# timohouben/GNN-XAI-TimeSeries-QualityControl

Hardware: AMD Instinct MI355X
Metric: ROC-AUC (5-fold CV) + train windows/sec, CML GCN at 1/2/4/8 MI355X (higher is better)
Workload: dtype bf16; 1 GPU; model=CML GCN (GeneralConv16+mean pool+LSTM TimeLayer f16 n_stacks2+dense64), global_batch=128, seq_len=181, parallelism=dp1, adjacency=radius(max_sample_distance=20), graph_steps=8, trainable_params=188193, hip_graph=True

## Files before the change

csrc/kernels/chain_head.h:

```cpp
#pragma once
#include "common.h"

namespace gq {

constexpr int CH_HU = 64;
constexpr int CH_AP = CH_HU + 4;
constexpr int CH_NW = 8;
constexpr int CH_WP = CH_HU + 4;

struct ChainHead {
  const float *W1, *b1, *W2, *b2, *W3, *b3;
  const float *y, *mask;
  float* logits;
  float* part;
  float* loss;
  double* sums;
  float* hist;
  int bins;
  int* ticket;
  int* done;
  int* ctl;
  int M;
  float alpha1, alpha2, w0, w1;
  const float* dloss;
  float* gpart;
  float *dW1, *db1, *dW2, *db2, *dW3, *db3;
};

template <int F>
struct ChainHeadRec {
  static constexpr int N = F * CH_HU + CH_HU + CH_HU * CH_HU + CH_HU + CH_HU + 1;
  static constexpr int PITCH = (N + 3) / 4 * 4;
};

typedef float ch_f4 __attribute__((ext_vector_type(4)));

__device__ __forceinline__ void ch_st(float* p, float v) {
  __hip_atomic_store(reinterpret_cast<unsigned*>(p), __float_as_uint(v), __ATOMIC_RELAXED, __HIP_MEMORY_SCOPE_AGENT);
}
__device__ __forceinline__ float ch_ld(const float* p) {
  return __uint_as_float(__hip_atomic_load(reinterpret_cast<const unsigned*>(p), __ATOMIC_RELAXED,
                                           __HIP_MEMORY_SCOPE_AGENT));
}

__device__ __forceinline__ float ch_leaky(float z, float a) { return z > 0.f ? z : a * z; }
__device__ __forceinline__ float ch_dleaky(float z, float a) { return z > 0.f ? 1.f : a; }

__device__ __forceinline__ int ch_tid() { return threadIdx.x & (64 * CH_NW - 1); }

__device__ __forceinline__ float ch_mask_sum(const float* __restrict__ mask, int M, float* red) {
  float s = 0.f;
  for (int i = ch_tid(); i < M; i += 64 * CH_NW) s += ch_ld(mask + i);
  s = wave_sum(s);
  if ((threadIdx.x & 63) == 0) red[ch_tid() >> 6] = s;
  __syncthreads();
  float t = 0.f;
#pragma unroll
  for (int k = 0; k < CH_NW; ++k) t += red[k];
  return t;
}

template <int NS>
__device__ __forceinline__ ch_f4 ch_mm_wk(const float* __restrict__ Wt, int ldw, int ot, int k0, const float* act,
                                          int lda) {
  const int l = threadIdx.x & 63, m = l & 15, kk = l >> 4;
  float a[NS];
#pragma unroll
  for (int s = 0; s < NS; ++s) a[s] = Wt[(size_t)(k0 + 4 * s + kk) * ldw + 16 * ot + m];
  ch_f4 acc = {0.f, 0.f, 0.f, 0.f};
#pragma unroll
  for (int s = 0; s < NS; ++s)
    acc = __builtin_amdgcn_mfma_f32_16x16x4f32(a[s], act[m * lda + k0 + 4 * s + kk], acc, 0, 0, 0);
  return acc;
}

template <int NS>
__device__ __forceinline__ ch_f4 ch_mm_wt(const float* __restrict__ W, int ldw, int ot, int k0, const float* act,
                                          int lda) {
  const int l = threadIdx.x & 63, m = l & 15, kk = l >> 4;
  float a[NS];
#pragma unroll
  for (int s = 0; s < NS; ++s) a[s] = W[(size_t)(16 * ot + m) * ldw + k0 + 4 * s + kk];
  ch_f4 acc = {0.f, 0.f, 0.f, 0.f};
#pragma unroll
  for (int s = 0; s < NS; ++s)
    acc = __builtin_amdgcn_mfma_f32_16x16x4f32(a[s], act[m * lda + k0 + 4 * s + kk], acc, 0, 0, 0);
  return acc;
}

__device__ __forceinline__ void ch_put(float* part, int lp, int ot, const ch_f4& d) {
  const int l = threadIdx.x & 63, n = l & 15, q = l >> 4;
#pragma unroll
// ... 29 lines not shown
  const int tid = ch_tid(), w = tid >> 6, j = tid & 63;
  const int ot = w & 3, kh = w >> 2;
  const float b1j = hd.b1[j], b2j = hd.b2[j];
  ch_put(part + kh * PT, CH_AP, ot, ch_mm_wk<F / 8>(sW1, CH_WP, ot, kh * (F / 2), hl, HLP));
  __syncthreads();
#pragma unroll
  for (int q = 0; q < 2; ++q) {
    const int r = w + 8 * q;
    const float z1 = b1j + part[r * CH_AP + j] + part[PT + r * CH_AP + j];
    if (sz1 != nullptr) sz1[r * CH_AP + j] = z1;
    sa1[r * CH_AP + j] = ch_leaky(z1, hd.alpha1);
  }
  __syncthreads();
  ch_put(part + kh * PT, CH_AP, ot, ch_mm_wk<8>(sW2, CH_WP, ot, kh * 32, sa1, CH_AP));
  __syncthreads();
#pragma unroll
  for (int q = 0; q < 2; ++q) {
    const int r = w + 8 * q;
    z2[q] = b2j + part[r * CH_AP + j] + part[PT + r * CH_AP + j];
  }
}

template <int F>
struct ChainHeadFwdLds {
  static constexpr int BYTES = (2 * 16 * CH_AP + 16 * CH_AP + 16 * 8 + (F + CH_HU) * CH_WP) * 4;
};

template <int F>
__device__ __forceinline__ float* ch_head_fwd_weights(char* scratch) {
  return reinterpret_cast<float*>(scratch) + 3 * 16 * CH_AP + 16 * 8;
}
template <int F>
__device__ __forceinline__ void chain_head_fwd_handoff(const ChainHead hd, int tile, int ntiles, char* scratch);
template <int F>
__device__ __forceinline__ void chain_head_fwd(const ChainHead hd, int tile, int ntiles, const float* hl, char* scratch,
                                               bool staged = false, bool handoff = true) {
  float* part = reinterpret_cast<float*>(scratch);
  float* sa1 = part + 2 * 16 * CH_AP;
  float* rowv = sa1 + 16 * CH_AP;
  float* sW1 = rowv + 16 * 8;
  float* sW2 = sW1 + F * CH_WP;
  if (!staged) ch_stage_weights<F>(hd, sW1, sW2);
  const int tid = threadIdx.x, w = tid >> 6, j = tid & 63;
  const float w3j = hd.W3[j], b3 = hd.b3[0];
  float yy[2], mm[2];
#pragma unroll
  for (int q = 0; q < 2; ++q) {
    const int rc = min(tile * 16 + w + 8 * q, hd.M - 1);
    yy[q] = ch_ld(hd.y + rc);
    mm[q] = ch_ld(hd.mask + rc);
  }
  float z2[2];
  ch_head_z2<F>(hd, sW1, sW2, hl, part, nullptr, sa1, z2);
#pragma unroll
  for (int q = 0; q < 2; ++q) {
    const int r = w + 8 * q, row = tile * 16 + r;
    const float z = wave_sum(ch_leaky(z2[q], hd.alpha2) * w3j) + b3;
    if (j == 0) {
      const bool valid = row < hd.M;
      const float m = valid ? mm[q] : 0.f, y = yy[q];
      if (valid && hd.logits != nullptr) hd.logits[row] = z;
      const float l = fmaxf(z, 0.f) - z * y + log1pf(__expf(-fabsf(z)));
      const float wc = y > 0.5f ? hd.w1 : hd.w0;
      const float p = sigmoidf_fast(z);
      const bool pos = y > 0.5f, pp = p > 0.5f;
      rowv[r * 8 + 0] = m * wc * l;
      rowv[r * 8 + 1] = m;
      rowv[r * 8 + 2] = (pp && pos) ? m : 0.f;
      rowv[r * 8 + 3] = (!pp && !pos) ? m : 0.f;
      rowv[r * 8 + 4] = (pp && !pos) ? m : 0.f;
      rowv[r * 8 + 5] = (!pp && pos) ? m : 0.f;
      if (hd.hist != nullptr && m != 0.f) {
        int b = (int)rintf(fminf(fmaxf(p, 0.f), 1.f) * (float)(hd.bins - 1));
        b = b < 0 ? 0 : (b >= hd.bins ? hd.bins - 1 : b);
        atomicAdd(&hd.hist[(pos ? hd.bins : 0) + b], m);
      }
    }
  }
  __syncthreads();
  if (handoff) chain_head_fwd_handoff<F>(hd, tile, ntiles, scratch);
}

template <int F>
__device__ __forceinline__ void chain_head_fwd_handoff(const ChainHead hd, int tile, int ntiles, char* scratch) {
  const float* rowv = reinterpret_cast<const float*>(scratch) + 3 * 16 * CH_AP;
  const int tid = threadIdx.x;
  if (tid < 6) {
    float s = 0.f;
#pragma unroll
    for (int k = 0; k < 16; ++k) s += rowv[k * 8 + tid];
    ch_st(hd.part + tile * 8 + tid, s);
  }
  asm volatile("s_waitcnt vmcnt(0)" ::: "memory");
  __syncthreads();
  if (tid == 0) {
    const int t = __hip_atomic_fetch_add(hd.ticket, 1, __ATOMIC_RELAXED, __HIP_MEMORY_SCOPE_AGENT);
    if (t == ntiles - 1) {
      double s[6] = {0, 0, 0, 0, 0, 0};
      for (int k = 0; k < ntiles; ++k)
        for (int q = 0; q < 6; ++q) s[q] += (double)ch_ld(hd.part + k * 8 + q);
      hd.loss[0] = (float)(s[0] / fmax(s[1], 1.0));
      if (hd.sums != nullptr)
        for (int q = 0; q < 6; ++q) hd.sums[q] += s[q];
      __hip_atomic_store(hd.ticket, 0, __ATOMIC_RELAXED, __HIP_MEMORY_SCOPE_AGENT);
    }
  }
}

template <int F>
struct ChainHeadBwdLds {
  static constexpr int BYTES = (16 * (F + 4) + 2 * 16 * CH_AP + 5 * 16 * CH_AP + 32 + (F + CH_HU) * CH_WP) * 4;
};

template <int F>
__device__ __forceinline__ void chain_head_bwd(const ChainHead hd, const float* __restrict__ hT, int tile, int ntiles,
                                               float* dh, char* scratch, int hld = -1, bool unit_gl = false,
                                               bool count = true, int nlive = 0, const float* pW1 = nullptr,
                                               const float* pW2 = nullptr) {
  constexpr int HLP = F + 4, PT = 16 * CH_AP;
  using Rec = ChainHeadRec<F>;
  float* sh = reinterpret_cast<float*>(scratch);
  float* part = sh + 16 * HLP;
  float* sz1 = part + 2 * PT;
  float* sa1 = sz1 + PT;
  float* sz2 = sa1 + PT;
  float* sad = sz2 + PT;
  float* sdz1 = sad + PT;
  float* misc = sdz1 + PT;
  float* sW1 = pW1 != nullptr ? const_cast<float*>(pW1) : misc + 32;
  float* sW2 = pW2 != nullptr ? const_cast<float*>(pW2) : sW1 + F * CH_WP;
  if (pW1 == nullptr) ch_stage_weights<F>(hd, sW1, sW2);
  const int tid = ch_tid(), w = tid >> 6, j = tid & 63;
  const int l = tid & 63, lm = l & 15, lq = l >> 4;
  const int row0 = tile * 16;
  const float* hsrc = hld < 0 ? hT + (size_t)row0 * F : hT;
  const int hp = hld < 0 ? F : hld;
  for (int e = tid; e < 16 * F / 4; e += 64 * CH_NW) {
    const int rr = 4 * e / F, k = 4 * e % F;
    const float4 v = *reinterpret_cast<const float4*>(hsrc + (size_t)rr * hp + k);
    *reinterpret_cast<float4*>(sh + rr * HLP + k) = v;
  }
  const float w3j = hd.W3[j], b3 = hd.b3[0], gl = unit_gl ? 1.f : hd.dloss[0];
  float yy[2], mm[2];
#pragma unroll
  for (int q = 0; q < 2; ++q) {
    const int rc = min(row0 + w + 8 * q, hd.M - 1);
    yy[q] = ch_ld(hd.y + rc);
    mm[q] = ch_ld(hd.mask + rc);
  }
  const float n = ch_mask_sum(hd.mask, hd.M, misc + 16);
  float z2[2];
  ch_head_z2<F>(hd, sW1, sW2, sh, part, sz1, sa1, z2);
#pragma unroll
  for (int q = 0; q < 2; ++q) {
    const int r = w + 8 * q;
    const float a2 = ch_leaky(z2[q], hd.alpha2);
    const float z = wave_sum(a2 * w3j) + b3;
    const float wc = yy[q] > 0.5f ? hd.w1 : hd.w0;
    const float d = (row0 + r < hd.M) ? gl / fmaxf(n, 1.f) * mm[q] * wc * (sigmoidf_fast(z) - yy[q]) : 0.f;
    sz2[r * CH_AP + j] = d * w3j * ch_dleaky(z2[q], hd.alpha2);
    sad[r * CH_AP + j] = a2 * d;
    if (j == 0) misc[r] = d;
  }
  __syncthreads();
  {
    const int ot = w & 3, kh = w >> 2;
    ch_put(part + kh * PT, CH_AP, ot, ch_mm_wt<8>(sW2, CH_WP, ot, kh * 32, sz2, CH_AP));
  }
  __syncthreads();
#pragma unroll
  for (int q = 0; q < 2; ++q) {
    const int r = w + 8 * q;
    const float da = part[r * CH_AP + j] + part[PT + r * CH_AP + j];
    sdz1[r * CH_AP + j] = da * ch_dleaky(sz1[r * CH_AP + j], hd.alpha1);
  }
  __syncthreads();
#pragma unroll
  for (int q = 0; q < F / 16 / CH_NW; ++q) {
    const int ot = w + CH_NW * q;
    ch_put(dh, HLP, ot, ch_mm_wt<16>(sW1, CH_WP, ot, 0, sdz1, CH_AP));
  }
  auto wgrad = [&](const float* a1, int lda1, int it, const float* a2, int jt) {
    ch_f4 acc = {0.f, 0.f, 0.f, 0.f};
#pragma unroll
    for (int s = 0; s < 4; ++s)
      acc = __builtin_amdgcn_mfma_f32_16x16x4f32(a1[(4 * s + lq) * lda1 + 16 * it + lm],
                                                 a2[(4 * s + lq) * CH_AP + 16 * jt + lm], acc, 0, 0, 0);
    return acc;
  };
  float* rec = hd.gpart + (size_t)tile * Rec::PITCH;
  float* rec2 = rec + F * CH_HU + CH_HU;
  const int wa = threadIdx.x >> 6, nwa = nlive > 0 ? nlive : (int)(blockDim.x >> 6);
  for (int t = wa; t < F / 16 * 4; t += nwa) {
    const int it = t >> 2, jt = t & 3;
    const ch_f4 acc = wgrad(sh, HLP, it, sdz1, jt);
#pragma unroll
    for (int k = 0; k < 4; ++k) ch_st(rec + (16 * it + 4 * lq + k) * CH_HU + 16 * jt + lm, acc[k]);
  }
  for (int t = wa; t < 16; t += nwa) {
    const int it = t >> 2, jt = t & 3;
    const ch_f4 acc = wgrad(sa1, CH_AP, it, sz2, jt);
#pragma unroll
    for (int k = 0; k < 4; ++k) ch_st(rec2 + (16 * it + 4 * lq + k) * CH_HU + 16 * jt + lm, acc[k]);
  }
  if (threadIdx.x < CH_HU) {
    float s1 = 0.f, s2 = 0.f, s3 = 0.f;
#pragma unroll
    for (int rr = 0; rr < 16; ++rr) {
      s1 += sdz1[rr * CH_AP + j];
      s2 += sz2[rr * CH_AP + j];
      s3 += sad[rr * CH_AP + j];
    }
    ch_st(rec + F * CH_HU + j, s1);
    ch_st(rec2 + CH_HU * CH_HU + j, s2);
    ch_st(rec2 + CH_HU * CH_HU + CH_HU + j, s3);
  } else if (threadIdx.x == CH_HU) {
    float s = 0.f;
#pragma unroll
    for (int rr = 0; rr < 16; ++rr) s += misc[rr];
    ch_st(rec2 + CH_HU * CH_HU + 2 * CH_HU, s);
  }
  if (!count) {
    __syncthreads();
    return;
  }
  asm volatile("s_waitcnt vmcnt(0)" ::: "memory");
  __syncthreads();
  if (threadIdx.x == 0) __hip_atomic_fetch_add(hd.ticket, 1, __ATOMIC_RELAXED, __HIP_MEMORY_SCOPE_AGENT);
}

template <int F>
__device__ __forceinline__ void chain_head_bwd_reduce(const ChainHead hd, int tile, int ntiles, bool pre = false,
                                                      float scale = 1.f) {
  using Rec = ChainHeadRec<F>;
  __shared__ int bad;
  if (threadIdx.x == 0 && pre) bad = 0;
  if (threadIdx.x == 0 && !pre) {
    int nap = 1, it = 0;
    bad = 0;
    while (__hip_atomic_load(hd.ticket, __ATOMIC_RELAXED, __HIP_MEMORY_SCOPE_AGENT) < ntiles) {
      for (int k = 0; k < nap; ++k) __builtin_amdgcn_s_sleep(8);
      nap = min(nap * 2, 8);
      if (++it > (1 << 22)) {
        __hip_atomic_store(hd.ctl + 2, 1, __ATOMIC_RELAXED, __HIP_MEMORY_SCOPE_AGENT);
        bad = 1;
        break;
      }
    }
  }
  __syncthreads();
  if (!bad) {
    const int chunk = (Rec::N + ntiles - 1) / ntiles;
    const int e1 = min(Rec::N, (tile + 1) * chunk);
    constexpr int RB = 4;
    for (int e0 = tile * chunk + (int)threadIdx.x; e0 < e1; e0 += RB * blockDim.x) {
      float acc[RB];
#pragma unroll
      for (int q = 0; q < RB; ++q) acc[q] = 0.f;
      for (int k = 0; k < ntiles; ++k) {
        float v[RB];
#pragma unroll
        for (int q = 0; q < RB; ++q) v[q] = ch_ld(hd.gpart + (size_t)k * Rec::PITCH + min(e0 + q * (int)blockDim.x, e1 - 1));
#pragma unroll
        for (int q = 0; q < RB; ++q) acc[q] += v[q];
      }
#pragma unroll
      for (int q = 0; q < RB; ++q) {
      const int e = e0 + q * (int)blockDim.x;
      if (e >= e1) break;
      const float s = acc[q] * scale;
      if (!isfinite(s)) __hip_atomic_store(hd.ctl + 7, 1, __ATOMIC_RELAXED, __HIP_MEMORY_SCOPE_AGENT);
      int o = e;
      if (o < F * CH_HU) { hd.dW1[o] += s; continue; }
      o -= F * CH_HU;
      if (o < CH_HU) { hd.db1[o] += s; continue; }
      o -= CH_HU;
      if (o < CH_HU * CH_HU) { hd.dW2[o] += s; continue; }
      o -= CH_HU * CH_HU;
      if (o < CH_HU) { hd.db2[o] += s; continue; }
      o -= CH_HU;
      if (o < CH_HU) { hd.dW3[o] += s; continue; }
      hd.db3[0] += s;
      }
    }
  }
  __syncthreads();
  if (threadIdx.x == 0) {
    const int d = __hip_atomic_fetch_add(hd.done, 1, __ATOMIC_ACQ_REL, __HIP_MEMORY_SCOPE_AGENT);
    if (d == ntiles - 1) {
      __hip_atomic_store(hd.ticket, 0, __ATOMIC_RELAXED, __HIP_MEMORY_SCOPE_AGENT);
      __hip_atomic_store(hd.done, 0, __ATOMIC_RELAXED, __HIP_MEMORY_SCOPE_AGENT);
    }
  }
}

}
```

csrc/kernels/lstm_chain.hip:

```cpp
#include "chain_head.h"
#include "common.h"
#include "gcn_fused.h"
#include "lstm_grads_body.h"
#include "lstm_tm_common.h"

#include <cstdlib>
#include <type_traits>

namespace gq {

typedef unsigned long long u64x2_t __attribute__((ext_vector_type(2)));
typedef unsigned u32x4_t __attribute__((ext_vector_type(4)));
typedef __bf16 bf16x2_t __attribute__((ext_vector_type(2)));

static constexpr int CHAIN_MAX = 8;
static constexpr int CHAIN_SPIN = 1 << 20;
#ifndef CHAIN_D
#define CHAIN_D 4
#endif
#ifndef CHAIN_D3
#define CHAIN_D3 2
#endif
#ifndef CHAIN_LEAD1
#define CHAIN_LEAD1 1
// ... 519 lines not shown
          stage_x((t + 1) & 1, 0, t + 1);
          if (iot == 0) chain_mark_wave(pr, t, 5);
          next_ld = t + 1 + D;
          if (iot == 0) chain_mark_wave(pr, t, 6);
        }
        kt = kt == 0 ? D - 1 : kt - 1;
        lds_barrier();
      }
    }
  } else {
    for (int t0 = 0; t0 < T; t0 += D) {
#pragma unroll
      for (int r = 0; r < D; ++r) {
        const int t = t0 + r;
        if (t >= T) break;
        compute_step(t, yes{}, (r + 1 == D) ? 0 : r + 1);
        if (own_pool && pooler && t >= 1) pool_step(t - 1);
        lds_barrier();
        chain_mark(pr, t, 3);
      }
    }
  }
  if constexpr (!IOW) {
    if (own_pool && pooler) pool_step(T - 1);
  }
}

struct ChainT4Lds {
  static constexpr int HS = 2 * 16 * (128 + 8) * 2;
  static constexpr int XS = 2 * 16 * (64 + 8) * 2;
  static constexpr int HL = 16 * (128 + 4) * 4;
  static constexpr int DHT = 16 * (128 + 4) * 4;
  static constexpr int HF = ChainHeadFwdLds<128>::BYTES;
  static constexpr int HB = DHT + ChainHeadBwdLds<128>::BYTES - (128 + CH_HU) * CH_WP * 4;
  static constexpr int BYTES = HS + XS + HL + HF + HB;
};

template <bool TRAIN>
__device__ __forceinline__ void chain_t4_stage(const ChainT4 Q, int tile, int ntiles, int Mp, unsigned tagb, int* ctl,
                                               char* smem) {
  constexpr int H = 128, G4 = 4 * H, NW = 16, CPL = 2, KX = 2, KSH = H / 32, HPB = H + 8, XP = 64 + 8;
  static_assert(ChainT4Lds::HS % 16 == 0 && ChainT4Lds::XS % 16 == 0 && ChainT4Lds::HL % 16 == 0, "t4 LDS layout");
  auto hs = reinterpret_cast<__bf16 (*)[16][HPB]>(smem);
  auto xs = reinterpret_cast<__bf16 (*)[16][XP]>(smem + ChainT4Lds::HS);
  float* hl = reinterpret_cast<float*>(smem + ChainT4Lds::HS + ChainT4Lds::XS);
  const int T = Q.T, Din = Q.Din, Dw = Q.Dw;
  const int tid = threadIdx.x, lane = tid & 63;
  const int w = __builtin_amdgcn_readfirstlane(tid >> 6);
  const int col = lane & 15, quad = lane >> 4;
  const int row0 = tile * 16;

  for (int i = tid; i < 2 * 16 * HPB; i += 1024) (&hs[0][0][0])[i] = (__bf16)0.0f;
  for (int i = tid; i < 2 * 16 * XP; i += 1024) (&xs[0][0][0])[i] = (__bf16)0.0f;
  const int n_el = 16 * Din;
  const bool own = tid < n_el;
  const int el = min(tid, n_el - 1), er = el / Din, ek = el % Din;
  const size_t xstep = (size_t)Mp * Din, xoff = (size_t)(row0 + er) * Din + ek;
  unsigned long long xq[3];
  auto load_x = [&](int tx) {
#pragma unroll
    for (int r = 0; r < 3; ++r) xq[r] = ld_granule(Q.xin + xoff + (size_t)(3 * tx + r) * xstep);
  };
  load_x(0);

  bf16x8_t ufr[CPL][KSH], wfr[CPL][KX];
  f32x4_t bias4[CPL];
  int unit[CPL];
// ... 114 lines not shown
}

__device__ __forceinline__ void chain_finish(int* ctl, int nblk) {
  if (threadIdx.x == 0) {
    const int old = __hip_atomic_fetch_add(ctl + 1, 1, __ATOMIC_RELAXED, __HIP_MEMORY_SCOPE_AGENT);
    if (old == nblk - 1) {
      __hip_atomic_store(ctl + 1, 0, __ATOMIC_RELAXED, __HIP_MEMORY_SCOPE_AGENT);
      __hip_atomic_store(ctl + 10, 0, __ATOMIC_RELAXED, __HIP_MEMORY_SCOPE_AGENT);
      __hip_atomic_fetch_add(ctl, 1, __ATOMIC_RELAXED, __HIP_MEMORY_SCOPE_AGENT);
    }
  }
}

static constexpr int CHAIN_LDS = ChainT4Lds::BYTES > CHAIN_LDS_STAGE ? ChainT4Lds::BYTES : CHAIN_LDS_STAGE;

template <bool TRAIN>
__global__ __launch_bounds__(1024) void lstm_chain_fwd_kernel(ChainArgs A) {
  const int nblk = gridDim.x;
  __shared__ __attribute__((aligned(16))) char smem[CHAIN_LDS];
  if ((int)blockIdx.x >= A.ns * A.nt8) {
    int r = (int)blockIdx.x - A.ns * A.nt8;
    if (A.t4.on) {
      if (r < A.nt8) {
        if (r < A.ntiles) {
          if (threadIdx.x == 0) A.trace[2 * blockIdx.x] = (long long)__builtin_amdgcn_s_memrealtime();
          const unsigned tagb = chain_tag_base((unsigned)__hip_atomic_load(A.ctl, __ATOMIC_RELAXED, __HIP_MEMORY_SCOPE_AGENT));
          constexpr int HOFF = ChainT4Lds::HS + ChainT4Lds::XS + ChainT4Lds::HL;
          float* hW1 = ch_head_fwd_weights<128>(smem + HOFF);
          ch_stage_weights<128>(A.t4.hd, hW1, hW1 + 128 * CH_WP);
          if (A.gp.on) {
            if (threadIdx.x == 0) chain_wait_count(A.ctl + 10, A.gp.Mp, A.ctl);
            __syncthreads();
          }
          chain_t4_stage<TRAIN>(A.t4, r, A.ntiles, A.Mp, tagb, A.ctl, smem);
          long long* mk = blockIdx.x < 64 ? A.trace + 512 + blockIdx.x : nullptr;
          if (mk != nullptr && threadIdx.x == 0) mk[0] = (long long)__builtin_amdgcn_s_memrealtime();
          if (threadIdx.x >= 64 * CH_NW) return;
          const bool pre = TRAIN && A.t4.hb != nullptr;
          chain_head_fwd<128>(A.t4.hd, r, A.ntiles, reinterpret_cast<const float*>(smem + ChainT4Lds::HS + ChainT4Lds::XS),
                              smem + HOFF, true, !pre);
          if (mk != nullptr && threadIdx.x == 0) mk[64] = (long long)__builtin_amdgcn_s_memrealtime();
          if constexpr (TRAIN) {
            if (A.t4.hb != nullptr) {
              __syncthreads();
              constexpr int OFF = HOFF + ChainT4Lds::HF;
              float* dhs = reinterpret_cast<float*>(smem + OFF);
              ChainHead hb = A.t4.hd;
              hb.gpart = A.t4.hb + (size_t)A.ntiles * 16 * 128;
              chain_head_bwd<128>(hb, reinterpret_cast<const float*>(smem + ChainT4Lds::HS + ChainT4Lds::XS), r, A.ntiles,
                                  dhs, smem + OFF + ChainT4Lds::DHT, 132, true, false, CH_NW, hW1, hW1 + 128 * CH_WP);
              for (int e = ch_tid(); e < 16 * 128; e += 64 * CH_NW)
                A.t4.hb[((size_t)r * 16 + e / 128) * 128 + e % 128] = dhs[(e / 128) * 132 + e % 128];
              chain_head_fwd_handoff<128>(A.t4.hd, r, A.ntiles, smem + HOFF);
            }
          }
          __syncthreads();
          if (threadIdx.x == 0) A.trace[2 * blockIdx.x + 1] = (long long)__builtin_amdgcn_s_memrealtime();
        }
        chain_finish(A.ctl, nblk);
        return;
      }
      r -= A.nt8;
    }
    if (r < A.npk) {
      const int f = r * 1024 + (int)threadIdx.x;
      if (A.pk != nullptr && f < T4PK_ALL) t4_pack_one(f, A.pkU, A.pkW, A.pkDw, A.pk);
    } else if (A.cf.on && r - A.npk < A.cf.Mp) {
      gcn_coef_fwd_body<2, 16>(A.cf, r - A.npk, smem);
    } else if (A.gp.on && r - A.npk - (A.cf.on ? A.cf.Mp : 0) < A.gp.Mp) {
      if (threadIdx.x == 0 && blockIdx.x < 256) A.trace[2 * blockIdx.x] = (long long)__builtin_amdgcn_s_memrealtime();
      const unsigned E = (unsigned)__hip_atomic_load(A.ctl, __ATOMIC_RELAXED, __HIP_MEMORY_SCOPE_AGENT);
      const int row = r - A.npk - (A.cf.on ? A.cf.Mp : 0);
      gcn_prod_body<2, 16>(A.gp, row, chain_tag_base(E), A.ctl + 10, smem, row < 32 ? A.trace + 640 + 4 * row : nullptr);
      if (threadIdx.x == 0 && blockIdx.x < 256) A.trace[2 * blockIdx.x + 1] = (long long)__builtin_amdgcn_s_memrealtime();
    }
    chain_finish(A.ctl, nblk);
    return;
  }
  const int s = blockIdx.x / A.nt8, tile = blockIdx.x % A.nt8;
  if (s >= A.ns || tile >= A.ntiles) {
    chain_finish(A.ctl, nblk);
    return;
  }
// ... 701 lines not shown
          const bf16x8_t bz = *reinterpret_cast<const bf16x8_t*>(&zs[p][col][32 * (kx * KPX + q) + 8 * quad]);
          b = __builtin_amdgcn_mfma_f32_16x16x32_bf16(ufk[q], bz, b, 0, 0, 0);
        }
#pragma unroll
        for (int r = 0; r < 4; ++r) {
          dpart[kg][col][16 * ut + 4 * quad + r] = a[r];
          xpart[p][kx][col][16 * xt + 4 * quad + r] = b[r];
        }
      }
      chain_mark(pr, s, 4);
      if constexpr (!PUBW) {
        const uint2 zv = *reinterpret_cast<const uint2*>(&zs[p][gz_seq][gz_c]);
        const int tz = t >= 0 ? t : T;
        *reinterpret_cast<uint2*>(zbase + (size_t)tz * zstep) = zv;
      }
      if constexpr (!PUBW) {
        const int ts = (s >= 1 && s <= T) ? t + 1 : T;
        store_dx(p ^ 1, ts, tagb | (unsigned)ts);
      }
      {
        lds_barrier();
        float sdh = 0.f;
#pragma unroll
        for (int g = 0; g < KG; ++g) sdh += dpart[g][col][unit];
        dhr = sdh;
      }
      chain_mark(pr, s, 5);
    }
  }
  __syncthreads();
  if constexpr (!PUBW) store_dx((T - 1) & 1, 0, tagb);
}

__device__ __forceinline__ void chain_t4_bwd_stage(const ChainT4B Q, int tile, int ntiles, int Mp, unsigned tagb,
                                                   char* smem, long long* mk = nullptr) {
  constexpr int H = 128, G4 = 4 * H, NW = 16, CPL = 2, HP = H + 4, ZP = G4 + 8, XP = 68;
  using L = ChainT4BLds;
  static_assert(L::DHT % 16 == 0 && L::ZS % 16 == 0 && L::DN % 16 == 0, "t4 backward LDS layout");
  float* dhT = reinterpret_cast<float*>(smem);
  char* rs = smem + L::DHT;
  auto zs = reinterpret_cast<__bf16 (*)[ZP]>(rs);
  auto dhn = reinterpret_cast<float (*)[16][HP]>(rs + L::ZS);
  auto dxp = reinterpret_cast<float (*)[16][XP]>(rs + L::ZS + L::DN);
  const int T = Q.T, Din = Q.Din, Dw = Q.Dw;
  const int tid = threadIdx.x, lane = tid & 63;
  const int w = __builtin_amdgcn_readfirstlane(tid >> 6);
  const int col = lane & 15, quad = lane >> 4;
  const int row0 = tile * 16;

  int unit[CPL];
  size_t so[CPL];
#pragma unroll
  for (int cc = 0; cc < CPL; ++cc) {
    const int gi = w + NW * cc;
    unit[cc] = 4 * gi + quad;
    so[cc] = (((size_t)tile * 8 + (gi & 7)) * 4 + (gi >> 3)) * 64 + lane;
  }
  const size_t sstep = (size_t)ntiles * 8 * 4 * 64;
  float4 rg[2][CPL];
  float2 rcs[2][CPL];
  auto load_slot = [&](int j, int t) {
    const size_t tc = (size_t)max(t, 0);
#pragma unroll
    for (int cc = 0; cc < CPL; ++cc) {
      const size_t o = tc * sstep + so[cc];
      rg[j][cc] = *reinterpret_cast<const float4*>(Q.g + o * 4);
      rcs[j][cc] = *reinterpret_cast<const float2*>(Q.c + o * 2);
    }
// ... 49 lines not shown
    load_slot(j, t - 2);
    lds_barrier();
    *reinterpret_cast<uint4*>(Q.dz + ((size_t)t * Mp + row0 + zq) * G4 + zc) = *reinterpret_cast<const uint4*>(&zs[zq][zc]);
    {
      f32x4_t a0 = {0.f, 0.f, 0.f, 0.f}, a1 = a0, b0 = a0, b1 = a0;
#pragma unroll
      for (int q = 0; q < 8; ++q) {
        const bf16x8_t bz = *reinterpret_cast<const bf16x8_t*>(&zs[col][32 * (8 * kh + q) + 8 * quad]);
        if (q & 1) a1 = __builtin_amdgcn_mfma_f32_16x16x32_bf16(ufr[q], bz, a1, 0, 0, 0);
        else a0 = __builtin_amdgcn_mfma_f32_16x16x32_bf16(ufr[q], bz, a0, 0, 0, 0);
      }
#pragma unroll
      for (int q = 0; q < 4; ++q) {
        const bf16x8_t bz = *reinterpret_cast<const bf16x8_t*>(&zs[col][32 * (4 * kq + q) + 8 * quad]);
        if (q & 1) b1 = __builtin_amdgcn_mfma_f32_16x16x32_bf16(wfr[q], bz, b1, 0, 0, 0);
        else b0 = __builtin_amdgcn_mfma_f32_16x16x32_bf16(wfr[q], bz, b0, 0, 0, 0);
      }
      const f32x4_t a = a0 + a1, b = b0 + b1;
#pragma unroll
      for (int r = 0; r < 4; ++r) {
        dhn[kh][col][16 * ut + 4 * quad + r] = a[r];
        dxp[kq][col][16 * dt + 4 * quad + r] = b[r];
      }
    }
    lds_barrier();
#pragma unroll
    for (int cc = 0; cc < CPL; ++cc) dhr[cc] = dhn[0][col][unit[cc]] + dhn[1][col][unit[cc]];
    const float v = (dxp[0][er][ek] + dxp[1][er][ek]) + (dxp[2][er][ek] + dxp[3][er][ek]);
    if (ownx) st_granule(Q.sout + xoff + (size_t)t * xstep, v, tagb | (unsigned)t);
  }
  }
  if (mk != nullptr && tid == 0) mk[64] = (long long)__builtin_amdgcn_s_memrealtime();
  if (Q.hb != nullptr) {
    ChainHead hd = Q.hd;
    hd.gpart = const_cast<float*>(Q.hb) + (size_t)ntiles * 16 * H;
    chain_head_bwd_reduce<H>(hd, tile, ntiles, true, Q.hd.dloss[0]);
  } else {
    chain_head_bwd_reduce<H>(Q.hd, tile, ntiles);
  }
}

__global__ __launch_bounds__(1024) void lstm_chain_bwd_kernel(ChainBArgs A) {
  const int nblk = gridDim.x;
  __shared__ __attribute__((aligned(16))) char smem[CHAINB_LDS];
  const int s = blockIdx.x / A.nt8, tile = blockIdx.x % A.nt8;
  if (s == A.ns && A.t4.on && tile < A.ntiles) {
    if (threadIdx.x == 0) A.trace[2 * blockIdx.x] = (long long)__builtin_amdgcn_s_memrealtime();
    const unsigned tagb = chain_tag_base((unsigned)__hip_atomic_load(A.ctl, __ATOMIC_RELAXED, __HIP_MEMORY_SCOPE_AGENT));
    chain_t4_bwd_stage(A.t4, tile, A.ntiles, A.Mp, tagb, smem, blockIdx.x < 64 ? A.trace + 512 + blockIdx.x : nullptr);
    __syncthreads();
    if (threadIdx.x == 0) A.trace[2 * blockIdx.x + 1] = (long long)__builtin_amdgcn_s_memrealtime();
    chain_finish(A.ctl, nblk);
    return;
  }
  if (s >= A.ns || tile >= A.ntiles) {
    chain_finish(A.ctl, nblk);
    return;
  }
  if (threadIdx.x == 0) A.trace[2 * blockIdx.x] = (long long)__builtin_amdgcn_s_memrealtime();
  const unsigned E = (unsigned)__hip_atomic_load(A.ctl, __ATOMIC_RELAXED, __HIP_MEMORY_SCOPE_AGENT);
  const unsigned tagb = chain_tag_base(E);
  const ChainBStage S = A.st[s];
  const int H = S.H, KX = S.KX;
  const bool src = s > 0 || A.t4.on;
#define GQ_CHAINB_STAGE_16(KXX, DD, SRCV, UPV, XOV) chain_bwd_stage16<KXX, DD, SRCV, UPV, XOV>
#define GQ_CHAINB_STAGE_32(KXX, DD, SRCV, UPV, XOV) chain_bwd_stage_sk<32, KXX, DD, SRCV, UPV, XOV>
#define GQ_CHAINB_STAGE_64(KXX, DD, SRCV, UPV, XOV) chain_bwd_stage_sk<64, KXX, DD, SRCV, UPV, XOV>
#define GQ_CHAINB_BODY3(HH, KXX, DD, SRCV, UPV, XOV)                                    \
  {                                                                                     \
    if (threadIdx.x >= chainb_live_threads(HH, TMC<HH>::NT)) return;                    \
    GQ_CHAINB_STAGE_##HH(KXX, DD, SRCV, UPV, XOV)(S, tile, A.ntiles, A.Mp, tagb, A.ctl, smem); \
  }
#define GQ_CHAINB_BODY2(HH, KXX, DD, SRCV, UPV)                                         \
  if (!SRCV || S.sout) GQ_CHAINB_BODY3(HH, KXX, DD, SRCV, UPV, true)                    \
  else GQ_CHAINB_BODY3(HH, KXX, DD, SRCV, UPV, false)
#define GQ_CHAINB_BODY(HH, KXX, DD)                                                     \
  {                                                                                     \
    if (src) { if (S.P > 0 && !S.punp) { GQ_CHAINB_BODY2(HH, KXX, DD, true, true) }    \
               else { GQ_CHAINB_BODY2(HH, KXX, DD, true, false) } }                     \
    else { if (S.P > 0) { GQ_CHAINB_BODY3(HH, KXX, DD, false, true, true) }             \
           else { GQ_CHAINB_BODY3(HH, KXX, DD, false, false, true) } }                  \
  }
// ... 228 lines not shown
    T = To;
    Din = H;
  }
  int nblk = ns * nt8;
  std::vector<at::Tensor> t4out;
  at::Tensor hb_t;
  if (t4 != nullptr) {
    TORCH_CHECK(pkW != nullptr && pkU != nullptr, "lstm_chain_head_fwd: time4 weights");
    check_f32_cuda(*t4->b, "bt4");
    const int Dw4 = (int)pkW->size(0);
    TORCH_CHECK(T >= 1 && T <= 16, "lstm_chain_head_fwd: time4 sequence length 1..16 (got ", T, ")");
    TORCH_CHECK(Din <= 64 && Dw4 >= 1 && Dw4 <= Din && t4->b->numel() == 512, "lstm_chain_head_fwd: time4 input width");
    ChainT4& Q = A.t4;
    Q.on = 1;
    Q.xin = reinterpret_cast<const unsigned long long*>(prev_stream.data_ptr<int64_t>());
    Q.W = pkW->data_ptr<float>();
    Q.U = pkU->data_ptr<float>();
    Q.b = t4->b->data_ptr<float>();
    at::Tensor h4 = at::empty({T, Mp, 128}, opt);
    at::Tensor g4 = train ? at::empty({(long)T * Mp * 128 * 4}, opt) : at::empty({0}, opt);
    at::Tensor c4 = train ? at::empty({(long)T * Mp * 128 * 2}, opt) : at::empty({0}, opt);
    Q.h = h4.data_ptr<float>();
    Q.g = train ? g4.data_ptr<float>() : nullptr;
    Q.c = train ? c4.data_ptr<float>() : nullptr;
    Q.T = T;
    Q.Din = Din;
    Q.Dw = Dw4;
    at::Tensor logits, loss, part;
    t4_head_fwd_args(Q.hd, t4->head, *t4->y, *t4->mask, t4->M, Mp, t4->alpha1, t4->alpha2, t4->w0, t4->w1, t4->sums,
                     t4->hist, logits, loss, part);
    t4out = {h4, g4, c4, logits, loss, part};
    const char* hbe = std::getenv("GNNQC_HEAD_BWD_IN_FWD");
    if (train && !(hbe != nullptr && hbe[0] == '0')) {
      hb_t = at::empty({(long)ntiles * 16 * 128 + (long)ntiles * ChainHeadRec<128>::PITCH}, opt);
      Q.hb = hb_t.data_ptr<float>();
    } else {
      hb_t = at::empty({0}, opt);
    }
    nblk += nt8;
  }
  at::Tensor pk;
  if (pkW != nullptr) {
    check_f32_cuda(*pkW, "Wt4");
    check_f32_cuda(*pkU, "Ut4");
    TORCH_CHECK(pkU->size(0) == 128 && pkU->size(1) == 512 && pkW->size(1) == 512 && pkW->size(0) <= 64,
                "lstm_chain_fwd_pack: time4 weights must be [<=64, 512] and [128, 512]");
    pk = at::empty({(long)T4PK_ALL * 4}, opt);
    A.pkU = pkU->data_ptr<float>();
    A.pkW = pkW->data_ptr<float>();
    A.pkDw = (int)pkW->size(0);
    A.pk = reinterpret_cast<bf16x8_t*>(pk.data_ptr<float>());
    A.npk = (T4PK_ALL + 1023) / 1024;
    nblk += A.npk;
    TORCH_CHECK(nblk <= chain_capacity(x.get_device()), "lstm_chain: ", nblk,
                " workgroups cannot all be resident on this device");
  }
  std::vector<at::Tensor> gp_keep;
  {
    const int dev = x.get_device();
    const GcnProdJob& P = gcn_pending(dev).prod;
    if (P.on) {
      const int H0 = A.st[0].H, Din0 = A.st[0].Din;
      const bool mine = train && t4 != nullptr && P.out == x.data_ptr<float>() && P.Mp == Mp &&
                        P.Cp == Din0 && P.D.T == (int)x.size(0) && Din0 % 2 == 0 &&
                        (H0 < 64 || 16 * Din0 / 2 <= 64 * TMC<64>::NW) &&
                        (long)P.D.T * Mp * Din0 * 8 < (1L << 31) && nblk + P.Mp <= chain_capacity(dev);
      if (mine) {
// ... 53 lines not shown
                                            at::TensorList head, const at::Tensor& y,
                                            const at::Tensor& mask, int64_t M, double alpha1, double alpha2, double w0,
                                            double w1, at::TensorList hgrads, at::TensorList g, at::TensorList c,
                                            at::TensorList W, at::TensorList U, at::TensorList pidx,
                                            at::IntArrayRef pool, at::IntArrayRef x_width, at::IntArrayRef T_in) {
  check_f32_cuda(x4, "x4");
  for (const at::Tensor* t : {&dloss, &h4, &g4, &c4, &Wt4, &Ut4}) check_f32_cuda(*t, "lstm_chain_head_bwd operand");
  TORCH_CHECK(x4.dim() == 3 && x4.is_contiguous(), "lstm_chain_head_bwd: x4 must be a contiguous [T4, Mp, Din]");
  const int T4 = (int)x4.size(0), Mp = (int)x4.size(1), Din = (int)x4.size(2), Dw = (int)Wt4.size(0);
  TORCH_CHECK(T4 >= 1 && T4 <= 16 && Din <= 64 && Dw >= 1 && Dw <= Din && Wt4.size(1) == 512 && Ut4.size(0) == 128 &&
                  Ut4.size(1) == 512, "lstm_chain_head_bwd: time4 shapes");
  TORCH_CHECK(dloss.numel() == 1, "lstm_chain_head_bwd: dloss must be a scalar");
  TORCH_CHECK(h4.numel() == (long)T4 * Mp * 128 && g4.numel() == (long)T4 * Mp * 128 * 4 && c4.numel() == (long)T4 * Mp * 128 * 2,
              "lstm_chain_head_bwd: time4 saved state shapes");
  TORCH_CHECK(pool.size() >= 1 && pool[0] == 3, "lstm_chain_head_bwd: the top chain stage must pool by 3");
  ChainBArgs A{};
  std::vector<at::Tensor> keep;
  c10::DeviceGuard guard(x4.device());
  auto opt = x4.options();
  at::Tensor so = at::empty({T4, Mp, Din}, opt.dtype(at::kLong));
  auto res = chain_bwd_setup(A, keep, x4, g, c, W, U, pidx, pool, x_width, T_in, (Mp / 16 + 7) / 8 * 8);
  A.st[0].dh = nullptr;
  A.st[0].din = reinterpret_cast<const unsigned long long*>(so.data_ptr<int64_t>());
  ChainT4B& Q = A.t4;
  Q.on = 1;
  Q.h = h4.data_ptr<float>();
  Q.g = g4.data_ptr<float>();
  Q.c = c4.data_ptr<float>();
  TORCH_CHECK(pk.is_cuda() && pk.is_contiguous() && pk.nbytes() == (size_t)T4PK_ALL * 16,
              "lstm_chain_head_bwd: pk must be the forward's full fragment image");
  Q.pk = reinterpret_cast<const bf16x8_t*>(pk.data_ptr());
  if (hb.numel() > 0) {
    check_f32_cuda(hb, "lstm_chain_head_bwd hb");
    TORCH_CHECK(hb.numel() == (long)(Mp / 16) * 16 * 128 + (long)(Mp / 16) * ChainHeadRec<128>::PITCH,
                "lstm_chain_head_bwd: hb must be the forward's precomputed head backward");
    Q.hb = hb.data_ptr<float>();
  } else {
    Q.hb = nullptr;
  }
  at::Tensor dz4 = at::empty({T4 + 1, Mp, 512}, opt.dtype(at::kBFloat16));
  Q.dz = bf16_ptr(dz4);
  Q.sout = reinterpret_cast<unsigned long long*>(so.data_ptr<int64_t>());
  Q.T = T4;
  Q.Din = Din;
  Q.Dw = Dw;
  at::Tensor gpart;
  t4_head_bwd_args(Q.hd, head, y, mask, M, Mp, alpha1, alpha2, w0, w1, dloss, hgrads, gpart);
  hipLaunchKernelGGL(lstm_chain_bwd_kernel, dim3((A.ns + 1) * A.nt8), dim3(1024), 0, stream(), A);
  GQ_LAUNCH_CHECK();
  res.insert(res.begin(), dz4);
  return res;
}

static std::vector<at::Tensor> chain_bwd_setup(ChainBArgs& A, std::vector<at::Tensor>& keep, const at::Tensor& dh,
                                               at::TensorList g, at::TensorList c, at::TensorList W, at::TensorList U,
                                               at::TensorList pidx, at::IntArrayRef pool, at::IntArrayRef x_width,
                                               at::IntArrayRef T_in, int extra_blocks) {
  check_f32_cuda(dh, "dh");
  const int ns = (int)W.size();
  TORCH_CHECK(ns >= 1 && ns <= CHAIN_MAX && (int)U.size() == ns && (int)g.size() == ns && (int)c.size() == ns &&
                  (int)pidx.size() == ns && (int)pool.size() == ns && (int)x_width.size() == ns &&
                  (int)T_in.size() == ns, "lstm_chain_bwd: stage lists");
  TORCH_CHECK(dh.dim() == 3 && dh.is_contiguous(), "lstm_chain_bwd: dh must be a contiguous [Ts, Mp, H]");
  const int Mp = (int)dh.size(1);
  TORCH_CHECK(Mp % 16 == 0, "lstm_chain_bwd: Mp");
  const int ntiles = Mp / 16, nt8 = (ntiles + 7) / 8 * 8;
  TORCH_CHECK(ns * nt8 + extra_blocks <= chain_capacity(dh.get_device()), "lstm_chain_bwd: ", ns * nt8 + extra_blocks,
              " workgroups cannot all be resident on this device");
// ... 105 lines not shown
```

Baseline: 548,800 train windows/s (whole job).

## Compute only head dh in forward, defer head weight-gradient records to backward

The forward kernel's precomputed head backward now reuses the forward activations (z, z2, sz1 kept in registers/LDS) to compute only dh, instead of rerunning a full head backward including weight-gradient records. The weight-gradient records are instead computed in the backward kernel's t4 stage through a noinline helper, followed by the normal reduction. This shortens the forward critical path and shrinks the hb buffer and LDS footprint, but moves the weight-gradient work back into the backward kernel.

```diff
diff --git a/csrc/kernels/chain_head.h b/csrc/kernels/chain_head.h
--- a/csrc/kernels/chain_head.h
+++ b/csrc/kernels/chain_head.h
@@ -48,16 +48,22 @@
 
 __device__ __forceinline__ int ch_tid() { return threadIdx.x & (64 * CH_NW - 1); }
 
-__device__ __forceinline__ float ch_mask_sum(const float* __restrict__ mask, int M, float* red) {
+__device__ __forceinline__ void ch_mask_partials(const float* __restrict__ mask, int M, float* red) {
   float s = 0.f;
   for (int i = ch_tid(); i < M; i += 64 * CH_NW) s += ch_ld(mask + i);
   s = wave_sum(s);
   if ((threadIdx.x & 63) == 0) red[ch_tid() >> 6] = s;
-  __syncthreads();
+}
+__device__ __forceinline__ float ch_mask_total(const float* red) {
   float t = 0.f;
 #pragma unroll
   for (int k = 0; k < CH_NW; ++k) t += red[k];
   return t;
+}
+__device__ __forceinline__ float ch_mask_sum(const float* __restrict__ mask, int M, float* red) {
+  ch_mask_partials(mask, M, red);
+  __syncthreads();
+  return ch_mask_total(red);
 }
 
 template <int NS>
@@ -153,9 +159,13 @@
 }
 template <int F>
 __device__ __forceinline__ void chain_head_fwd_handoff(const ChainHead hd, int tile, int ntiles, char* scratch);
+struct ChainHeadKeep {
+  float z2[2], z[2], yy[2], mm[2];
+};
 template <int F>
 __device__ __forceinline__ void chain_head_fwd(const ChainHead hd, int tile, int ntiles, const float* hl, char* scratch,
-                                               bool staged = false, bool handoff = true) {
+                                               bool staged = false, bool handoff = true, float* sz1 = nullptr,
+                                               ChainHeadKeep* keep = nullptr) {
   float* part = reinterpret_cast<float*>(scratch);
   float* sa1 = part + 2 * 16 * CH_AP;
   float* rowv = sa1 + 16 * CH_AP;
@@ -172,11 +182,17 @@
     mm[q] = ch_ld(hd.mask + rc);
   }
   float z2[2];
-  ch_head_z2<F>(hd, sW1, sW2, hl, part, nullptr, sa1, z2);
+  ch_head_z2<F>(hd, sW1, sW2, hl, part, sz1, sa1, z2);
 #pragma unroll
   for (int q = 0; q < 2; ++q) {
     const int r = w + 8 * q, row = tile * 16 + r;
     const float z = wave_sum(ch_leaky(z2[q], hd.alpha2) * w3j) + b3;
+    if (keep != nullptr) {
+      keep->z2[q] = z2[q];
+      keep->z[q] = z;
+      keep->yy[q] = yy[q];
+      keep->mm[q] = mm[q];
+    }
     if (j == 0) {
       const bool valid = row < hd.M;
       const float m = valid ? mm[q] : 0.f, y = yy[q];
@@ -228,6 +244,69 @@
   }
 }
 
+__device__ __forceinline__ float ch_head_d(const ChainHead& hd, bool valid, float gl, float n, float z, float y, float m) {
+  const float wc = y > 0.5f ? hd.w1 : hd.w0;
+  return valid ? gl / fmaxf(n, 1.f) * m * wc * (sigmoidf_fast(z) - y) : 0.f;
+}
+
+template <int F>
+__device__ __forceinline__ void ch_head_dh(const ChainHead& hd, const float d[2], const float z2[2], float w3j,
+                                           const float* sW1, const float* sW2, float* part, const float* sz1,
+                                           float* sz2, float* sdz1, float* dh) {
+  constexpr int HLP = F + 4, PT = 16 * CH_AP;
+  const int tid = ch_tid(), w = tid >> 6, j = tid & 63;
+#pragma unroll
+  for (int q = 0; q < 2; ++q) sz2[(w + 8 * q) * CH_AP + j] = d[q] * w3j * ch_dleaky(z2[q], hd.alpha2);
+  __syncthreads();
+  {
+    const int ot = w & 3, kh = w >> 2;
+    ch_put(part + kh * PT, CH_AP, ot, ch_mm_wt<8>(sW2, CH_WP, ot, kh * 32, sz2, CH_AP));
+  }
+  __syncthreads();
+#pragma unroll
+  for (int q = 0; q < 2; ++q) {
+    const int r = w + 8 * q;
+    const float da = part[r * CH_AP + j] + part[PT + r * CH_AP + j];
+    sdz1[r * CH_AP + j] = da * ch_dleaky(sz1[r * CH_AP + j], hd.alpha1);
+  }
+  __syncthreads();
+#pragma unroll
+  for (int q = 0; q < F / 16 / CH_NW; ++q) {
+    const int ot = w + CH_NW * q;
+    ch_put(dh, HLP, ot, ch_mm_wt<16>(sW1, CH_WP, ot, 0, sdz1, CH_AP));
+  }
+}
+
+template <int F>
+struct ChainHeadDhLds {
+  static constexpr int BYTES = 3 * 16 * CH_AP * 4;
+};
+template <int F>
+__device__ __forceinline__ float* ch_head_dh_sz1(char* dhscratch) { return reinterpret_cast<float*>(dhscratch); }
+template <int F>
+__device__ __forceinline__ float* ch_head_dh_red(char* dhscratch) {
+  return reinterpret_cast<float*>(dhscratch) + 2 * 16 * CH_AP;
+}
+
+template <int F>
+__device__ __forceinline__ void chain_head_dh(const ChainHead hd, int tile, const ChainHeadKeep& keep, char* fscratch,
+                                              char* dhscratch, float* dh) {
+  float* part = reinterpret_cast<float*>(fscratch);
+  const float* sW1 = ch_head_fwd_weights<F>(fscratch);
+  const float* sW2 = sW1 + F * CH_WP;
+  float* sz1 = ch_head_dh_sz1<F>(dhscratch);
+  float* sz2 = sz1 + 16 * CH_AP;
+  float* sdz1 = sz2 + 16 * CH_AP;
+  const int tid = ch_tid(), w = tid >> 6, j = tid & 63;
+  const float w3j = hd.W3[j];
+  const float n = ch_mask_total(ch_head_dh_red<F>(dhscratch));
+  float d[2];
+#pragma unroll
+  for (int q = 0; q < 2; ++q)
+    d[q] = ch_head_d(hd, tile * 16 + w + 8 * q < hd.M, 1.f, n, keep.z[q], keep.yy[q], keep.mm[q]);
+  ch_head_dh<F>(hd, d, keep.z2, w3j, sW1, sW2, part, sz1, sz2, sdz1, dh);
+}
+
 template <int F>
 struct ChainHeadBwdLds {
   static constexpr int BYTES = (16 * (F + 4) + 2 * 16 * CH_AP + 5 * 16 * CH_AP + 32 + (F + CH_HU) * CH_WP) * 4;
@@ -235,9 +314,7 @@
 
 template <int F>
 __device__ __forceinline__ void chain_head_bwd(const ChainHead hd, const float* __restrict__ hT, int tile, int ntiles,
-                                               float* dh, char* scratch, int hld = -1, bool unit_gl = false,
-                                               bool count = true, int nlive = 0, const float* pW1 = nullptr,
-                                               const float* pW2 = nullptr) {
+                                               float* dh, char* scratch) {
   constexpr int HLP = F + 4, PT = 16 * CH_AP;
   using Rec = ChainHeadRec<F>;
   float* sh = reinterpret_cast<float*>(scratch);
@@ -248,20 +325,18 @@
   float* sad = sz2 + PT;
   float* sdz1 = sad + PT;
   float* misc = sdz1 + PT;
-  float* sW1 = pW1 != nullptr ? const_cast<float*>(pW1) : misc + 32;
-  float* sW2 = pW2 != nullptr ? const_cast<float*>(pW2) : sW1 + F * CH_WP;
-  if (pW1 == nullptr) ch_stage_weights<F>(hd, sW1, sW2);
+  float* sW1 = misc + 32;
+  float* sW2 = sW1 + F * CH_WP;
+  ch_stage_weights<F>(hd, sW1, sW2);
   const int tid = ch_tid(), w = tid >> 6, j = tid & 63;
   const int l = tid & 63, lm = l & 15, lq = l >> 4;
   const int row0 = tile * 16;
-  const float* hsrc = hld < 0 ? hT + (size_t)row0 * F : hT;
-  const int hp = hld < 0 ? F : hld;
   for (int e = tid; e < 16 * F / 4; e += 64 * CH_NW) {
     const int rr = 4 * e / F, k = 4 * e % F;
-    const float4 v = *reinterpret_cast<const float4*>(hsrc + (size_t)rr * hp + k);
+    const float4 v = *reinterpret_cast<const float4*>(hT + (size_t)(row0 + rr) * F + k);
     *reinterpret_cast<float4*>(sh + rr * HLP + k) = v;
   }
-  const float w3j = hd.W3[j], b3 = hd.b3[0], gl = unit_gl ? 1.f : hd.dloss[0];
+  const float w3j = hd.W3[j], b3 = hd.b3[0], gl = hd.dloss[0];
   float yy[2], mm[2];
 #pragma unroll
   for (int q = 0; q < 2; ++q) {
@@ -270,37 +345,18 @@
     mm[q] = ch_ld(hd.mask + rc);
   }
   const float n = ch_mask_sum(hd.mask, hd.M, misc + 16);
-  float z2[2];
+  float z2[2], d[2];
   ch_head_z2<F>(hd, sW1, sW2, sh, part, sz1, sa1, z2);
 #pragma unroll
   for (int q = 0; q < 2; ++q) {
     const int r = w + 8 * q;
     const float a2 = ch_leaky(z2[q], hd.alpha2);
     const float z = wave_sum(a2 * w3j) + b3;
-    const float wc = yy[q] > 0.5f ? hd.w1 : hd.w0;
-    const float d = (row0 + r < hd.M) ? gl / fmaxf(n, 1.f) * mm[q] * wc * (sigmoidf_fast(z) - yy[q]) : 0.f;
-    sz2[r * CH_AP + j] = d * w3j * ch_dleaky(z2[q], hd.alpha2);
-    sad[r * CH_AP + j] = a2 * d;
-    if (j == 0) misc[r] = d;
-  }
-  __syncthreads();
-  {
-    const int ot = w & 3, kh = w >> 2;
-    ch_put(part + kh * PT, CH_AP, ot, ch_mm_wt<8>(sW2, CH_WP, ot, kh * 32, sz2, CH_AP));
-  }
-  __syncthreads();
-#pragma unroll
-  for (int q = 0; q < 2; ++q) {
-    const int r = w + 8 * q;
-    const float da = part[r * CH_AP + j] + part[PT + r * CH_AP + j];
-    sdz1[r * CH_AP + j] = da * ch_dleaky(sz1[r * CH_AP + j], hd.alpha1);
-  }
-  __syncthreads();
-#pragma unroll
-  for (int q = 0; q < F / 16 / CH_NW; ++q) {
-    const int ot = w + CH_NW * q;
-    ch_put(dh, HLP, ot, ch_mm_wt<16>(sW1, CH_WP, ot, 0, sdz1, CH_AP));
-  }
+    d[q] = ch_head_d(hd, row0 + r < hd.M, gl, n, z, yy[q], mm[q]);
+    sad[r * CH_AP + j] = a2 * d[q];
+    if (j == 0) misc[r] = d[q];
+  }
+  ch_head_dh<F>(hd, d, z2, w3j, sW1, sW2, part, sz1, sz2, sdz1, dh);
   auto wgrad = [&](const float* a1, int lda1, int it, const float* a2, int jt) {
     ch_f4 acc = {0.f, 0.f, 0.f, 0.f};
 #pragma unroll
@@ -311,7 +367,7 @@
   };
   float* rec = hd.gpart + (size_t)tile * Rec::PITCH;
   float* rec2 = rec + F * CH_HU + CH_HU;
-  const int wa = threadIdx.x >> 6, nwa = nlive > 0 ? nlive : (int)(blockDim.x >> 6);
+  const int wa = threadIdx.x >> 6, nwa = (int)(blockDim.x >> 6);
   for (int t = wa; t < F / 16 * 4; t += nwa) {
     const int it = t >> 2, jt = t & 3;
     const ch_f4 acc = wgrad(sh, HLP, it, sdz1, jt);
@@ -341,22 +397,16 @@
     for (int rr = 0; rr < 16; ++rr) s += misc[rr];
     ch_st(rec2 + CH_HU * CH_HU + 2 * CH_HU, s);
   }
-  if (!count) {
-    __syncthreads();
-    return;
-  }
   asm volatile("s_waitcnt vmcnt(0)" ::: "memory");
   __syncthreads();
   if (threadIdx.x == 0) __hip_atomic_fetch_add(hd.ticket, 1, __ATOMIC_RELAXED, __HIP_MEMORY_SCOPE_AGENT);
 }
 
 template <int F>
-__device__ __forceinline__ void chain_head_bwd_reduce(const ChainHead hd, int tile, int ntiles, bool pre = false,
-                                                      float scale = 1.f) {
+__device__ __forceinline__ void chain_head_bwd_reduce(const ChainHead hd, int tile, int ntiles) {
   using Rec = ChainHeadRec<F>;
   __shared__ int bad;
-  if (threadIdx.x == 0 && pre) bad = 0;
-  if (threadIdx.x == 0 && !pre) {
+  if (threadIdx.x == 0) {
     int nap = 1, it = 0;
     bad = 0;
     while (__hip_atomic_load(hd.ticket, __ATOMIC_RELAXED, __HIP_MEMORY_SCOPE_AGENT) < ntiles) {
@@ -389,7 +439,7 @@
       for (int q = 0; q < RB; ++q) {
       const int e = e0 + q * (int)blockDim.x;
       if (e >= e1) break;
-      const float s = acc[q] * scale;
+      const float s = acc[q];
       if (!isfinite(s)) __hip_atomic_store(hd.ctl + 7, 1, __ATOMIC_RELAXED, __HIP_MEMORY_SCOPE_AGENT);
       int o = e;
       if (o < F * CH_HU) { hd.dW1[o] += s; continue; }
diff --git a/csrc/kernels/lstm_chain.hip b/csrc/kernels/lstm_chain.hip
--- a/csrc/kernels/lstm_chain.hip
+++ b/csrc/kernels/lstm_chain.hip
@@ -575,7 +575,7 @@
   static constexpr int HL = 16 * (128 + 4) * 4;
   static constexpr int DHT = 16 * (128 + 4) * 4;
   static constexpr int HF = ChainHeadFwdLds<128>::BYTES;
-  static constexpr int HB = DHT + ChainHeadBwdLds<128>::BYTES - (128 + CH_HU) * CH_WP * 4;
+  static constexpr int HB = DHT + ChainHeadDhLds<128>::BYTES;
   static constexpr int BYTES = HS + XS + HL + HF + HB;
 };
 
@@ -756,23 +756,23 @@
             if (threadIdx.x == 0) chain_wait_count(A.ctl + 10, A.gp.Mp, A.ctl);
             __syncthreads();
           }
+          const bool pre = TRAIN && A.t4.hb != nullptr;
+          constexpr int OFF = HOFF + ChainT4Lds::HF;
+          char* dhscr = smem + OFF + ChainT4Lds::DHT;
+          if (pre) ch_mask_partials(A.t4.hd.mask, A.t4.hd.M, ch_head_dh_red<128>(dhscr));
           chain_t4_stage<TRAIN>(A.t4, r, A.ntiles, A.Mp, tagb, A.ctl, smem);
           long long* mk = blockIdx.x < 64 ? A.trace + 512 + blockIdx.x : nullptr;
           if (mk != nullptr && threadIdx.x == 0) mk[0] = (long long)__builtin_amdgcn_s_memrealtime();
           if (threadIdx.x >= 64 * CH_NW) return;
-          const bool pre = TRAIN && A.t4.hb != nullptr;
+          ChainHeadKeep keep;
           chain_head_fwd<128>(A.t4.hd, r, A.ntiles, reinterpret_cast<const float*>(smem + ChainT4Lds::HS + ChainT4Lds::XS),
-                              smem + HOFF, true, !pre);
+                              smem + HOFF, true, !pre, pre ? ch_head_dh_sz1<128>(dhscr) : nullptr, &keep);
           if (mk != nullptr && threadIdx.x == 0) mk[64] = (long long)__builtin_amdgcn_s_memrealtime();
           if constexpr (TRAIN) {
             if (A.t4.hb != nullptr) {
+              float* dhs = reinterpret_cast<float*>(smem + OFF);
+              chain_head_dh<128>(A.t4.hd, r, keep, smem + HOFF, dhscr, dhs);
               __syncthreads();
-              constexpr int OFF = HOFF + ChainT4Lds::HF;
-              float* dhs = reinterpret_cast<float*>(smem + OFF);
-              ChainHead hb = A.t4.hd;
-              hb.gpart = A.t4.hb + (size_t)A.ntiles * 16 * 128;
-              chain_head_bwd<128>(hb, reinterpret_cast<const float*>(smem + ChainT4Lds::HS + ChainT4Lds::XS), r, A.ntiles,
-                                  dhs, smem + OFF + ChainT4Lds::DHT, 132, true, false, CH_NW, hW1, hW1 + 128 * CH_WP);
               for (int e = ch_tid(); e < 16 * 128; e += 64 * CH_NW)
                 A.t4.hb[((size_t)r * 16 + e / 128) * 128 + e % 128] = dhs[(e / 128) * 132 + e % 128];
               chain_head_fwd_handoff<128>(A.t4.hd, r, A.ntiles, smem + HOFF);
@@ -1540,8 +1540,18 @@
   if constexpr (!PUBW) store_dx((T - 1) & 1, 0, tagb);
 }
 
-__device__ __forceinline__ void chain_t4_bwd_stage(const ChainT4B Q, int tile, int ntiles, int Mp, unsigned tagb,
-                                                   char* smem, long long* mk = nullptr) {
+typedef __attribute__((address_space(4))) ChainBArgs ChainBKernArgs;
+typedef __attribute__((address_space(3))) char ChainLdsChar;
+__device__ __noinline__ void chain_t4_bwd_records(const ChainBKernArgs* ka, ChainLdsChar* smem, int tile, int ntiles,
+                                                  int Mp) {
+  using L = ChainT4BLds;
+  char* s = (char*)smem;
+  const ChainT4B& Q = ((const ChainBArgs*)ka)->t4;
+  chain_head_bwd<128>(Q.hd, Q.h + (size_t)(Q.T - 1) * Mp * 128, tile, ntiles, reinterpret_cast<float*>(s), s + L::DHT);
+}
+
+__device__ __forceinline__ void chain_t4_bwd_stage(const ChainT4B Q, const ChainBKernArgs* kargs, int tile, int ntiles,
+                                                   int Mp, unsigned tagb, char* smem, long long* mk = nullptr) {
   constexpr int H = 128, G4 = 4 * H, NW = 16, CPL = 2, HP = H + 4, ZP = G4 + 8, XP = 68;
   using L = ChainT4BLds;
   static_assert(L::DHT % 16 == 0 && L::ZS % 16 == 0 && L::DN % 16 == 0, "t4 backward LDS layout");
@@ -1657,12 +1667,10 @@
   }
   if (mk != nullptr && tid == 0) mk[64] = (long long)__builtin_amdgcn_s_memrealtime();
   if (Q.hb != nullptr) {
-    ChainHead hd = Q.hd;
-    hd.gpart = const_cast<float*>(Q.hb) + (size_t)ntiles * 16 * H;
-    chain_head_bwd_reduce<H>(hd, tile, ntiles, true, Q.hd.dloss[0]);
-  } else {
-    chain_head_bwd_reduce<H>(Q.hd, tile, ntiles);
-  }
+    __syncthreads();
+    chain_t4_bwd_records(kargs, (ChainLdsChar*)smem, tile, ntiles, Mp);
+  }
+  chain_head_bwd_reduce<H>(Q.hd, tile, ntiles);
 }
 
 __global__ __launch_bounds__(1024) void lstm_chain_bwd_kernel(ChainBArgs A) {
@@ -1672,7 +1680,8 @@
   if (s == A.ns && A.t4.on && tile < A.ntiles) {
     if (threadIdx.x == 0) A.trace[2 * blockIdx.x] = (long long)__builtin_amdgcn_s_memrealtime();
     const unsigned tagb = chain_tag_base((unsigned)__hip_atomic_load(A.ctl, __ATOMIC_RELAXED, __HIP_MEMORY_SCOPE_AGENT));
-    chain_t4_bwd_stage(A.t4, tile, A.ntiles, A.Mp, tagb, smem, blockIdx.x < 64 ? A.trace + 512 + blockIdx.x : nullptr);
+    chain_t4_bwd_stage(A.t4, (const ChainBKernArgs*)__builtin_amdgcn_kernarg_segment_ptr(), tile, A.ntiles, A.Mp, tagb,
+                       smem, blockIdx.x < 64 ? A.trace + 512 + blockIdx.x : nullptr);
     __syncthreads();
     if (threadIdx.x == 0) A.trace[2 * blockIdx.x + 1] = (long long)__builtin_amdgcn_s_memrealtime();
     chain_finish(A.ctl, nblk);
@@ -1967,7 +1976,7 @@
     t4out = {h4, g4, c4, logits, loss, part};
     const char* hbe = std::getenv("GNNQC_HEAD_BWD_IN_FWD");
     if (train && !(hbe != nullptr && hbe[0] == '0')) {
-      hb_t = at::empty({(long)ntiles * 16 * 128 + (long)ntiles * ChainHeadRec<128>::PITCH}, opt);
+      hb_t = at::empty({(long)ntiles * 16 * 128}, opt);
       Q.hb = hb_t.data_ptr<float>();
     } else {
       hb_t = at::empty({0}, opt);
@@ -2087,8 +2096,7 @@
   Q.pk = reinterpret_cast<const bf16x8_t*>(pk.data_ptr());
   if (hb.numel() > 0) {
     check_f32_cuda(hb, "lstm_chain_head_bwd hb");
-    TORCH_CHECK(hb.numel() == (long)(Mp / 16) * 16 * 128 + (long)(Mp / 16) * ChainHeadRec<128>::PITCH,
-                "lstm_chain_head_bwd: hb must be the forward's precomputed head backward");
+    TORCH_CHECK(hb.numel() == (long)(Mp / 16) * 16 * 128, "lstm_chain_head_bwd: hb must be the forward's dh tiles");
     Q.hb = hb.data_ptr<float>();
   } else {
     Q.hb = nullptr;
```

After: 560,800 train windows/s (whole job), median of 6. +2.2%, better.
